# zengxianyu/sketchedit

Measured on AMD Instinct MI355X. Metric: images/sec, higher is better.
Workload: dtype f32; 1 GPU; SketchEdit inference forward (netM+netG, use_cam, pool max) 256x256 batch 32 per GPU, procedural weights; global_batch=32, size=256, per_gpu_batch=32, execution=default, two streams

## Files before the change

### sketchedit_amd/_lib.py

```python
import contextlib
import ctypes
import os
import subprocess
import threading

import numpy as np

_HERE = os.path.dirname(os.path.abspath(__file__))
LIB_PATH = os.environ.get("SKETCHEDIT_HIP_LIB") or os.path.join(_HERE, "lib", "libsketchedit_hip.so")
CSRC = os.path.join(_HERE, "csrc")
SOURCES = ["se_gconv.hip", "se_rconv16.hip", "se_rconv96.hip", "se_rtile.hip", "se_rtilew.hip", "se_wino.hip", "se_wino24.hip", "se_wino48.hip", "se_wino_up.hip", "se_wino_up48.hip", "se_attention.hip", "se_att_stream.hip", "se_misc.hip", "se_resize.hip",
           "se_window.hip", "se_feather.hip", "se_fill.hip", "se_select.hip", "se_lasso.hip", "se_modify.hip", "se_outline.hip", "se_move.hip", "se_warp.hip", "se_filter.hip", "se_adjust.hip", "se_png.hip", "se_jpg.hip", "se_pack.hip",
           "se_plan.hip", "se_api_window.hip", "se_api_select.hip", "se_api_move.hip", "se_api_codec.hip", "se_api_debug.hip", "se_api.hip"]

SE_NET_G, SE_NET_M = 0, 1
RESAMPLE_LANCZOS, RESAMPLE_BILINEAR, RESAMPLE_BICUBIC = 1, 2, 3
FLAG_USE_CAM, FLAG_POOL_MAX, FLAG_NO_MASK_CC, FLAG_NO_MASK_COARSE, FLAG_JOINT_TRAIN_INP = 1, 2, 4, 8, 16
FLAG_LOW_LATENCY, FLAG_GRAPH, FLAG_PACKED_OUT, FLAG_BF16, FLAG_CONSERVATIVE = 32, 64, 128, 256, 512
LOW_LATENCY_MAX_PIXELS = 3 * 256 * 256
LOW_LATENCY_MAX_SINGLE_IMAGE = 512 * 512

SYMBOLS = ["se_create", "se_destroy", "se_last_error", "se_version", "se_load_weights", "se_weights_ready",
           "se_workspace_bytes", "se_netM_forward", "se_netM_forward_ex", "se_netG_forward", "se_netG_forward_taps", "se_inference", "se_inference_u8", "se_gated_conv2d",
           "se_gated_conv2d_ex", "se_attention", "se_attention_ex", "se_quantize_u8", "se_dequantize_u8", "se_inference_u8io", "se_profile_enable",
# ... 301 lines not shown
        if device not in _shared:
            _shared[device] = Engine(device)
        return _shared[device]


def set_option(name, value):
    if load_library().se_debug_set_option(name.encode(), int(value)):
        raise SketchEditHipError("unknown developer switch %r" % name)


def get_option(name):
    v = ctypes.c_int(0)
    if load_library().se_debug_get_option(name.encode(), ctypes.byref(v)):
        raise SketchEditHipError("unknown developer switch %r" % name)
    return v.value


def reset_options():
    load_library().se_debug_reset_options()


def gconv_form(cin, cout, H, W, k=3, stride=1, rate=1, act="elu", upsample=False, cin1=0, x1_is_vector=False, B=1,
               low_latency=False, bf16=False, conservative=False, net=SE_NET_G):
    flags = (FLAG_LOW_LATENCY if low_latency else 0) | (FLAG_BF16 if bf16 else 0) | (FLAG_CONSERVATIVE if conservative else 0)
    buf = ctypes.create_string_buffer(64)
    fn = load_library().se_debug_gconv_form
    fn.argtypes, fn.restype = [ctypes.c_int] * 14 + [ctypes.c_char_p, ctypes.c_size_t], ctypes.c_int
    if fn(cin, cin1, int(bool(x1_is_vector)), cout, k, stride, rate, {"elu": 0, "relu": 1, None: 2}[act],
          int(bool(upsample)), B, H, W, flags, net, buf, len(buf)):
        raise SketchEditHipError("gconv_form: not a layer gated_conv2d takes")
    return buf.value.decode().split(",")


def flags_from_opt(opt):
    f = 0
    if getattr(opt, "use_cam", False):
        f |= FLAG_USE_CAM
    pool = getattr(opt, "pool_type", "avg")
    if pool == "max":
        f |= FLAG_POOL_MAX
    elif pool != "avg":
        raise NotImplementedError(pool)
    if getattr(opt, "no_mask_cc", False):
        f |= FLAG_NO_MASK_CC
    if getattr(opt, "no_mask_coarse", False):
        f |= FLAG_NO_MASK_COARSE
    if getattr(opt, "joint_train_inp", False):
        f |= FLAG_JOINT_TRAIN_INP
    return f


def _ptr(t):
    return None if t is None else ctypes.c_void_p(t.data_ptr())


def _check_dev(*ts):
    import torch
    for t in ts:
        if t is None:
            continue
        if not (isinstance(t, torch.Tensor) and t.is_cuda and t.dtype == torch.float32 and t.is_contiguous()):
            raise SketchEditHipError("expected contiguous float32 CUDA(HIP) tensors")


def upload_u8(a, device):
    import warnings
# ... 1070 lines not shown
```

### sketchedit_amd/csrc/se_api.hip

```cpp
#include "se_host.h"

using namespace se;

namespace se {

thread_local std::string g_create_err;

}

namespace {

void destroy_graph(se_ctx::GraphEntry& g) {
  if (g.exec) {
    if (g.stream) (void)hipStreamSynchronize(g.stream);
    (void)hipGraphExecDestroy(g.exec);
  }
  if (g.graph) (void)hipGraphDestroy(g.graph);
  g.exec = nullptr; g.graph = nullptr;
}
void drop_graphs(se_ctx* c) {
  for (auto& g : c->graphs) destroy_graph(g);
  c->graphs.clear();
}
void evict_lru_graph(se_ctx* c) {
// ... 46 lines not shown
  }
  t.last_use = ++c->rs_clock;
  c->rs_tables.push_back(std::move(t));
  return &c->rs_tables.back();
}

unsigned char* rs_scratch(se_ctx* c, size_t bytes) {
  if (bytes > c->rs_scratch_bytes) {
    if (c->rs_scratch) {
      (void)hipStreamSynchronize(c->rs_stream);
      (void)hipFree(c->rs_scratch);
      c->rs_scratch = nullptr; c->rs_scratch_bytes = 0;
    }
    const size_t sz = (bytes + ((size_t)1 << 20) - 1) & ~(((size_t)1 << 20) - 1);
    if (hipMalloc(&c->rs_scratch, sz) != hipSuccess) { c->rs_scratch = nullptr; fail(c, "resize: cannot allocate %zu bytes", sz); return nullptr; }
    c->rs_scratch_bytes = sz;
  }
  return c->rs_scratch;
}

int inference_u8_locked(se_ctx* c, void* stream, const float* image, const float* sketch, unsigned char* rgb_out,
                        unsigned char* mask_u8_out, void* ws, size_t ws_bytes, int B, int H, int W, int flags, int tail_planes,
                        const unsigned char* lock8) {
  flags &= ~(SE_FLAG_GRAPH | SE_FLAG_PACKED_OUT);
  const size_t plane = ((size_t)B * H * W * 4 + 255) & ~(size_t)255;
  const size_t tail = (2 + (size_t)tail_planes) * plane;
  if (ws_bytes < tail) return fail(c, "workspace too small: %zu bytes", ws_bytes);
  float* hard_all = (float*)((char*)ws + ws_bytes - tail + plane);
  float* soft_all = (float*)((char*)ws + ws_bytes - tail);
  const size_t HW = (size_t)H * W;
  const int nb = pass_size(c, B, H, W, flags);
  if (!nb) return 1;
  if (poison(c, soft_all, 2 * plane, (hipStream_t)stream)) return 1;
  for (int b0 = 0; b0 < B; b0 += nb) {
    const int bb = std::min(nb, B - b0);
    const se_ctx::Peaks pk = plan_peaks(c, 3, bb, H, W, flags, false);
    if (carve(c, pk, ws, ws_bytes, tail)) return 1;
    const float *img = image + b0 * 3 * HW, *sk = sketch + b0 * HW;
    float *hard = hard_all + b0 * HW, *soft = soft_all + b0 * HW;
    begin_call(c, stream, flags);
    int rc = plan_netM(c, img, sk, soft, hard, nullptr, bb, H, W, 0, lock8 ? lock8 + b0 * HW : nullptr);
    if (rc) return rc;
    if (carve(c, pk, ws, ws_bytes, tail)) return 1;
    c->rgb8 = rgb_out + b0 * 3 * HW; c->m8 = mask_u8_out ? mask_u8_out + b0 * HW : nullptr;
    rc = plan_netG(c, img, img, hard, hard, sk, nullptr, nullptr, soft, nullptr, bb, H, W, flags);
    if (rc) return rc;
  }
  return 0;
}

}

namespace {

int resize_locked(se_ctx* c, hipStream_t st, const unsigned char* in, int B, int Hin, int Win, int C, ResizeOut o, int Hout,
                  int Wout, int filter) {
  if (!in || (o.mode == RESIZE_OUT_U8 ? !o.u8 : !o.f32)) return fail(c, "null pointer argument");
  if (B < 1 || B > 65535 || Hin < 1 || Win < 1 || Hout < 1 || Wout < 1 || Hin > 65535 || Hout > 65535 || (C != 1 && C != 3))
    return fail(c, "resize: bad shape B=%d %dx%dx%d -> %dx%d (C in {1, 3}, heights and B < 65536)", B, Hin, Win, C, Hout, Wout);
  if (filter != SE_RESAMPLE_BILINEAR && filter != SE_RESAMPLE_BICUBIC && filter != SE_RESAMPLE_LANCZOS)
    return fail(c, "resize: unsupported filter %d", filter);
  if (o.mode == RESIZE_OUT_IMAGE_F32) o.lut = c->lut8;
  if (rs_enter(c, st)) return 1;
  set_profiler(&c->prof);
  o.H = Hout; o.W = Wout;
  const bool need_h = Win != Wout, need_v = Hin != Hout;
  if (!need_h && !need_v) {
    if (o.mode == RESIZE_OUT_U8) {
      HIPCHK(c, hipMemcpyAsync(o.u8, in, (size_t)B * Hin * Win * C, hipMemcpyDeviceToDevice, st));
      return 0;
    }
    if (((size_t)Hin * Win) % 4 || ((uintptr_t)in & 3) || ((uintptr_t)o.f32 & 15))
      return fail(c, "resize: an unresized fp32 output needs H W %% 4 == 0, a 4-byte aligned input and a 16-byte aligned output");
    if (o.mode == RESIZE_OUT_IMAGE_F32 && C == 3)
      HIPCHK(c, launch_dequantize_u8(in, nullptr, c->lut8, o.f32, nullptr, B, Hin, Win, st));
    else if (o.mode == RESIZE_OUT_SKETCH_F32 && C == 1)
      HIPCHK(c, launch_dequantize_u8(nullptr, in, c->lut8, nullptr, o.f32, B, Hin, Win, st));
    else
// ... 139 lines not shown
}

int se_weights_ready(se_ctx* c) {
  if (!c) return 0;
  std::lock_guard<std::mutex> lk(c->mu);
  for (auto* net : {&c->G, &c->M})
    for (auto& kv : *net)
      if (!kv.second.packed) return 0;
  return 1;
}

size_t se_workspace_bytes(se_ctx* c, int B, int H, int W) {
  if (!c) return 0;
  std::lock_guard<std::mutex> lk(c->mu);
  if (check_dims(c, B, H, W)) return 0;
  c->fork2 = opt(OPT_FORK_DEFAULT) != 0;
  size_t peak = 0;
  for (int cam = 0; cam < 2; ++cam)
    for (int joint = 0; joint < 2; ++joint)
      for (int ll = 0; ll < 2; ++ll)
        for (int bf = 0; bf < 2; ++bf) {
          const int flags = (cam ? SE_FLAG_USE_CAM : 0) | (joint ? SE_FLAG_JOINT_TRAIN_INP : 0) | (ll ? SE_FLAG_LOW_LATENCY : 0) |
                            (bf ? SE_FLAG_BF16 : 0) | SE_FLAG_POOL_MAX;
          const int nb = pass_size(c, B, H, W, flags);
          if (!nb) return 0;
          const int last = B % nb;
          for (int ser = 0; ser < 2; ++ser)
            for (int mi = 0; mi < 2; ++mi)
              for (int bb : {nb, last}) {
                if (!bb) continue;
                c->serial = ser != 0;
                const se_ctx::Peaks pk = plan_peaks(c, 3, bb, H, W, flags, mi != 0);
                if (pk.main + pk.side > peak) peak = pk.main + pk.side;
              }
          c->serial = false;
        }
  return peak + 6 * (((size_t)B * H * W * 4 + 255) & ~(size_t)255);
}

int se_netM_forward_ex(se_ctx* c, void* stream, const float* image, const float* sketch, float* mask_out,
                       float* maskim_out, void* ws, size_t ws_bytes, int B, int H, int W, int exec_flags) {
  if (!c) return 1;
  std::lock_guard<std::mutex> lk(c->mu);
  if (check_dims(c, B, H, W)) return 1;
  if (!image || !sketch || !mask_out || !ws) return fail(c, "null pointer argument");
  if (forward_enter(c)) return 1;
  exec_flags &= SE_FLAG_LOW_LATENCY | SE_FLAG_BF16 | SE_FLAG_CONSERVATIVE;
  const int nb = pass_size(c, B, H, W, exec_flags);
  if (!nb) return 1;
  const size_t HW = (size_t)H * W;
  for (int b0 = 0; b0 < B; b0 += nb) {
    const int bb = std::min(nb, B - b0);
    if (carve(c, plan_peaks(c, 1, bb, H, W, exec_flags, maskim_out != nullptr), ws, ws_bytes, 0)) return 1;
    begin_call(c, stream, exec_flags);
    const int rc = plan_netM(c, image + b0 * 3 * HW, sketch + b0 * HW, mask_out + b0 * HW, nullptr,
                             maskim_out ? maskim_out + b0 * 3 * HW : nullptr, bb, H, W);
    if (rc) return rc;
  }
  return 0;
}

int se_netM_forward(se_ctx* c, void* stream, const float* image, const float* sketch, float* mask_out,
                    float* maskim_out, void* ws, size_t ws_bytes, int B, int H, int W) {
  return se_netM_forward_ex(c, stream, image, sketch, mask_out, maskim_out, ws, ws_bytes, B, H, W, 0);
}

// ... 11 lines not shown
  const size_t HW = (size_t)H * W;
  for (int b0 = 0; b0 < B; b0 += nb) {
    const int bb = std::min(nb, B - b0);
    if (carve(c, plan_peaks(c, 2, bb, H, W, flags, false), ws, ws_bytes, 0)) return 1;
    begin_call(c, stream, flags);
    c->taps = taps;
    const int rc = plan_netG(c, x + b0 * 3 * HW, x2 + b0 * 3 * HW, mask + b0 * HW, mask2 + b0 * HW, guide + b0 * HW,
                             coarse_out ? coarse_out + b0 * 3 * HW : nullptr, fine_out + b0 * 3 * HW, nullptr, nullptr, bb, H, W, flags);
    c->taps = nullptr;
    if (rc) return rc;
  }
  return 0;
}

int se_netG_forward(se_ctx* c, void* stream, const float* x, const float* x2, const float* mask, const float* mask2,
                    const float* guide, float* coarse_out, float* fine_out, void* ws, size_t ws_bytes, int B, int H,
                    int W, int flags) {
  return se_netG_forward_taps(c, stream, x, x2, mask, mask2, guide, coarse_out, fine_out, ws, ws_bytes, B, H, W, flags, nullptr);
}

namespace {
int enqueue_inference(se_ctx* c, void* stream, const float* image, const float* sketch, float* composed_out, float* mask_out,
                      float* hard_out, float* maskim_out, float* coarse_out, float* fine_out, void* ws, size_t ws_bytes,
                      int B, int H, int W, int flags, const unsigned char* lock8 = nullptr) {
  const size_t plane = ((size_t)B * H * W * 4 + 255) & ~(size_t)255;
  float* hard_all = hard_out ? hard_out : (float*)((char*)ws + ws_bytes - plane);
  const size_t HW = (size_t)H * W;
  const long packed_bs = (flags & SE_FLAG_PACKED_OUT) ? 4l * H * W : 0;
  if (packed_bs) mask_out = composed_out + 3 * HW;
  const size_t comp_bs = packed_bs ? (size_t)packed_bs : 3 * HW, mask_bs = packed_bs ? (size_t)packed_bs : HW;
  const int nb = pass_size(c, B, H, W, flags);
  if (!nb) return 1;
  if (!hard_out && poison(c, hard_all, plane, (hipStream_t)stream)) return 1;
  for (int b0 = 0; b0 < B; b0 += nb) {
    const int bb = std::min(nb, B - b0);
    const se_ctx::Peaks pk = plan_peaks(c, 3, bb, H, W, flags, maskim_out != nullptr);
    if (carve(c, pk, ws, ws_bytes, plane)) return 1;
    const float *img = image + b0 * 3 * HW, *sk = sketch + b0 * HW;
    float *hard = hard_all + b0 * HW, *mk = mask_out + b0 * mask_bs;
    begin_call(c, stream, flags);
    int rc = plan_netM(c, img, sk, mk, hard, maskim_out ? maskim_out + b0 * 3 * HW : nullptr, bb, H, W, packed_bs,
                       lock8 ? lock8 + b0 * HW : nullptr);
    if (rc) return rc;
    if (carve(c, pk, ws, ws_bytes, plane)) return 1;
    rc = plan_netG(c, img, img, hard, hard, sk, coarse_out ? coarse_out + b0 * 3 * HW : nullptr, fine_out ? fine_out + b0 * 3 * HW : nullptr,
                   mk, composed_out + b0 * comp_bs, bb, H, W, flags, packed_bs);
    if (rc) return rc;
  }
  return 0;
}
}

int se_inference(se_ctx* c, void* stream, const float* image, const float* sketch, float* composed_out,
                 float* mask_out, float* hard_out, float* maskim_out, float* coarse_out, float* fine_out, void* ws,
                 size_t ws_bytes, int B, int H, int W, int flags) {
  if (!c) return 1;
  std::lock_guard<std::mutex> lk(c->mu);
  if (check_dims(c, B, H, W)) return 1;
  if (!image || !sketch || !composed_out || (!mask_out && !(flags & SE_FLAG_PACKED_OUT)) || !ws) return fail(c, "null pointer argument");
  if (forward_enter(c)) return 1;
  if (!(flags & SE_FLAG_GRAPH) || c->prof.on || poison_byte() != 0)
    return enqueue_inference(c, stream, image, sketch, composed_out, mask_out, hard_out, maskim_out, coarse_out, fine_out, ws,
                             ws_bytes, B, H, W, flags);
  const std::vector<long long> key = {(long long)(size_t)image, (long long)(size_t)sketch, (long long)(size_t)composed_out,
                                      (long long)(size_t)mask_out, (long long)(size_t)hard_out, (long long)(size_t)maskim_out,
                                      (long long)(size_t)coarse_out, (long long)(size_t)fine_out, (long long)(size_t)ws,
                                      (long long)ws_bytes, B, H, W, flags, opt_epoch()};
  se_ctx::GraphEntry* ge = nullptr;
  for (auto& g : c->graphs)
    if (g.key == key) { ge = &g; break; }
  if (!ge) {
    if (c->graphs.size() >= 16) evict_lru_graph(c);
    c->graphs.emplace_back();
    c->graphs.back().key = key;
    c->graphs.back().last_use = ++c->graph_clock;
    return enqueue_inference(c, stream, image, sketch, composed_out, mask_out, hard_out, maskim_out, coarse_out, fine_out, ws,
                             ws_bytes, B, H, W, flags);
  }
  ge->last_use = ++c->graph_clock;
// ... 165 lines not shown
```

### sketchedit_amd/csrc/se_api_debug.hip

```cpp
#include "se_host.h"

using namespace se;

extern "C" {

int se_profile_enable(se_ctx* c, int on) {
  if (!c) return 1;
  std::lock_guard<std::mutex> lk(c->mu);
  HIPCHK(c, hipSetDevice(c->device));
  c->prof.recs.clear();
  c->prof.used = 0;
  if (on && c->prof.pool.empty()) {
    c->prof.pool.resize(2 * 1024);
    for (auto& e : c->prof.pool) HIPCHK(c, hipEventCreate(&e));
  }
  c->prof.on = on != 0;
  return 0;
}

int se_profile_report(se_ctx* c, char* buf, size_t cap) {
  if (!c || !buf || cap < 64) return 1;
  std::lock_guard<std::mutex> lk(c->mu);
  HIPCHK(c, hipSetDevice(c->device));
  HIPCHK(c, hipDeviceSynchronize());
// ... 20 lines not shown
  std::map<std::string, long> cnt;
  for (auto& r : c->prof.recs) {
    if (!r.name) continue;
    float t = 0.f;
    if (hipEventElapsedTime(&t, r.a, r.b) != hipSuccess) continue;
    std::string k = std::string(prof_label_name(r.label)) + ":" + r.name;
    if (!cnt.count(k)) keys.push_back(k);
    agg[k].first += t; agg[k].second += r.flops; aggx[k] += r.exec_flops; cnt[k]++;
  }
  first = true;
  for (auto& k : keys) {
    char t[384];
    snprintf(t, sizeof t, "%s{\"layer\": \"%s\", \"launches\": %ld, \"total_ms\": %.6f, \"flops\": %.6e, \"flops_executed\": %.6e}",
             first ? "" : ", ", k.c_str(), cnt[k], agg[k].first, agg[k].second, aggx[k]);
    s += t;
    first = false;
  }
  s += "], \"launches\": [";
  first = true;
  for (auto& r : c->prof.recs) {
    char t[256];
    snprintf(t, sizeof t, "%s{\"form\": \"%s\", \"kernel\": \"%s\", \"layer\": \"%s\", \"workgroups\": %ld}", first ? "" : ", ",
             r.form ? r.form : "?", prof_label_name(r.label), r.name ? r.name : "", r.blocks);
    s += t;
    first = false;
  }
  s += "]}";
  if (s.size() + 1 > cap) return fail(c, "profile buffer too small");
  memcpy(buf, s.c_str(), s.size() + 1);
  return 0;
}

int se_debug_set_option(const char* name, int value) { return opt_set(name, value); }
int se_debug_get_option(const char* name, int* value) { return opt_get(name, value); }
void se_debug_reset_options(void) { opt_reset(); }

int se_debug_gconv_form(int cin, int cin1, int src1_is_vector, int cout, int k, int stride, int rate, int act, int upsample,
                        int B, int H, int W, int exec_flags, int net_id, char* out, size_t cap) {
  if (!out || cin <= 0 || cin1 < 0 || cout <= 0 || k <= 0 || stride <= 0 || rate <= 0 || B <= 0 || H <= 0 || W <= 0) return 1;
  const bool bf = (exec_flags & SE_FLAG_BF16) != 0;
  const int gran = bf ? 8 : 4;
  if (cin1 && ((cin % gran) || (cin1 % gran))) return 1;
  const LayerDef d = {"test", cin + cin1, cout, k, stride, rate, act, upsample};
  const bool raw = small_layer(d);
  if (raw && (k != 3 || cin != 12 || cin1 || (cout != 1 && cout != 3) || stride != 1 || rate != 1 || upsample)) return 1;
  if (!raw && (cout % 8)) return 1;
  const LayerFacts f = layer_facts(d, cin + cin1);
  if (!raw && f.cfg < 0) return 1;
  const int Cp = (cin + gran - 1) & ~(gran - 1);
  if (!raw && Cp + cin1 != f.CG[bf] * gran) return 1;
  const bool vec = cin1 && src1_is_vector;
  const ConvCall q = {d, f, B, H, W, Cp, cin1, cin1 ? (vec ? SRC2_VECTOR : SRC2_TENSOR) : SRC2_NONE, bf,
                      (exec_flags & SE_FLAG_LOW_LATENCY) != 0, (exec_flags & SE_FLAG_CONSERVATIVE) != 0, net_id, vec};
  const Choice ch = choose_form(q);
  const char* name = form_name(ch, q);
  if (!name) return 1;
  const std::string s = std::string(ch.fold ? "vecbias," : "") + name;
  if (s.size() + 1 > cap) return 1;
  memcpy(out, s.c_str(), s.size() + 1);
  return 0;
}

int se_gated_conv2d_ex(se_ctx* c, void* stream, const float* x, const float* x1, int x1_is_vector, const float* w_host,
                       const float* b_host, float* y, int B, int Cin, int Cin1, int H, int W, int Cout, int k, int stride,
                       int rate, int act, int upsample, int exec_flags) {
  if (!c || !x || !w_host || !b_host || !y) return 1;
  std::lock_guard<std::mutex> lk(c->mu);
// ... 202 lines not shown
```

### sketchedit_amd/csrc/se_host.h

```cpp
#pragma once
#include "../../include/sketchedit_hip.h"
#include "se_kernels.h"
#include "se_pack.h"

#include <cstdarg>
#include <cstdint>
#include <cstdlib>
#include <cstdio>
#include <cstring>
#include <algorithm>
#include <map>
#include <mutex>
#include <numeric>
#include <string>
#include <vector>

namespace se {

struct Arena {
  struct Blk { size_t off, size; bool used; };
  std::vector<Blk> blks;
  size_t cap = 0, peak = 0;
  bool dry = false;
  char* base = nullptr;
// ... 26 lines not shown
    for (size_t i = 0; i < blks.size(); ++i) {
      if (blks[i].off == off && blks[i].used) {
        blks[i].used = false;
        if (i + 1 < blks.size() && !blks[i + 1].used) { blks[i].size += blks[i + 1].size; blks.erase(blks.begin() + i + 1); }
        if (i > 0 && !blks[i - 1].used) { blks[i - 1].size += blks[i].size; blks.erase(blks.begin() + i); }
        return;
      }
    }
  }
};

}

struct se_ctx {
  int device = 0;
  std::mutex mu;
  std::string err;
  std::map<std::string, se::Layer> G, M;
  se::Layer wconv1_j4;
  float* zeros = nullptr;
  float* lut8 = nullptr;
  se::Arena arena;
  se::Arena arena2;
  hipStream_t st = nullptr;
  hipStream_t st_main = nullptr;
  hipStream_t st_side = nullptr;
  hipEvent_t ev_fork = nullptr, ev_join = nullptr;
  bool dry = false;
  bool low_latency = false;
  int cur_net = SE_NET_G;
  bool bf16 = false;
  bool serial = false;
  bool fork2 = true;
  bool conservative = false;
  const se_netG_taps* taps = nullptr;
  float* vbias_ws = nullptr;
  const float* vec32 = nullptr;
  unsigned char* rgb8 = nullptr;
  unsigned char* m8 = nullptr;
  se::Profiler prof;
  struct Peaks { size_t main, side; };
  std::map<std::vector<long long>, Peaks> peaks;
  size_t dry_max_act = 0;
  std::map<std::vector<long long>, long long> act_per_img;
  struct GraphEntry {
    std::vector<long long> key;
    hipGraph_t graph = nullptr;
    hipGraphExec_t exec = nullptr;
    hipStream_t stream = nullptr;
    unsigned long long last_use = 0;
  };
  unsigned long long graph_clock = 0;
  std::vector<GraphEntry> graphs;
  struct ResampleTable {
    int in, out, filter, ksize;
    std::vector<int> host;
    int* dev = nullptr;
    unsigned long long last_use = 0;
  };
  std::vector<ResampleTable> rs_tables;
  unsigned long long rs_clock = 0;
  unsigned char* rs_scratch = nullptr;
  size_t rs_scratch_bytes = 0;
  hipStream_t rs_stream = nullptr;
  bool rs_used = false;
  hipEvent_t rs_event = nullptr;
// ... 36 lines not shown
inline int poison_byte() {
  const int v = opt(OPT_TEST_POISON);
  return v >= 1 && v <= 255 ? v : 0;
}
inline int poison(se_ctx* c, void* p, size_t bytes, hipStream_t st) {
  const int v = poison_byte();
  if (!v || !p || !bytes) return 0;
  HIPCHK(c, hipMemsetAsync(p, v, bytes, st));
  return 0;
}

inline bool aligned_to(const void* p, int a) { return ((uintptr_t)p & (uintptr_t)(a - 1)) == 0; }

inline size_t pad256(size_t n) { return (n + 255) & ~(size_t)255; }

inline bool overlaps(const void* a, size_t an, const void* b, size_t bn) {
  return (uintptr_t)a < (uintptr_t)b + bn && (uintptr_t)b < (uintptr_t)a + an;
}

inline int check_dims(se_ctx* c, int B, int H, int W) {
  if (B < 1 || H < 16 || W < 16 || (H % 8) || (W % 8)) return fail(c, "bad shape B=%d H=%d W=%d (H, W must be multiples of 8, >= 16)", B, H, W);
  return 0;
}

inline void begin_call(se_ctx* c, void* stream, int flags) {
  c->st = c->st_main = (hipStream_t)stream;
  c->dry = false;
  c->low_latency = (flags & SE_FLAG_LOW_LATENCY) != 0;
  c->bf16 = (flags & SE_FLAG_BF16) != 0;
  c->conservative = (flags & SE_FLAG_CONSERVATIVE) != 0;
  c->serial = c->prof.on;
  c->taps = nullptr;
  c->rgb8 = nullptr; c->m8 = nullptr;
  c->cur_net = SE_NET_G;
  set_profiler(&c->prof);
}

inline int forward_enter(se_ctx* c) {
  HIPCHK(c, hipSetDevice(c->device));
  c->serial = c->prof.on;
  c->fork2 = opt(OPT_FORK_DEFAULT) != 0;
  return 0;
}

inline int device_enter(se_ctx* c) {
  HIPCHK(c, hipSetDevice(c->device));
  set_profiler(&c->prof);
  return 0;
}

extern const LayerDef G_LAYERS[], M_LAYERS[];
extern const int NG, NM;

int run_gconv(se_ctx* c, const Layer& L, const float* src0, int C0, const float* src1, int C1, int src1_vec, float* dst,
              int B, int Hin, int Win);

struct Act {
  float* p = nullptr;
  int H = 0, W = 0, C = 0;
};

struct Plan {
  se_ctx* c;
  std::map<std::string, Layer>& net;
  int B;
  int rc = 0;
  Arena* ar;
  Plan(se_ctx* c_, std::map<std::string, Layer>& n, int B_) : c(c_), net(n), B(B_), ar(&c_->arena) {}
  float* alloc_raw(size_t nfloats) {
    float* p = ar->alloc(nfloats);
    if (!p && !rc) rc = fail(c, "workspace too small (need more than %zu bytes)", ar->cap);
    if (p && !rc && !c->dry && poison(c, p, (nfloats * 4 + 255) & ~(size_t)255, c->st)) rc = 1;
    return p;
  }
  Act alloc(int H, int W, int C) {
    Act a; a.H = H; a.W = W;
    if (c->bf16) {
      a.C = (C + 7) & ~7;
      a.p = alloc_raw(((size_t)B * H * W * a.C + 1) / 2);
    } else {
      a.C = C;
      a.p = alloc_raw((size_t)B * H * W * C);
    }
    if (c->dry) c->dry_max_act = std::max(c->dry_max_act, (size_t)B * H * W * a.C * (c->bf16 ? 2 : 4));
    return a;
  }
  void release(const float* p) {
    if (!p) return;
    if (c->arena2.owns(p)) c->arena2.release(p); else c->arena.release(p);
  }
  void free(Act& a) { release(a.p); a.p = nullptr; }
  bool forked() const { return (c->low_latency || (c->fork2 && !c->serial)) && c->st_side; }
  int side_begin() {
    if (!forked()) return 0;
    ar = &c->arena2;
    if (c->dry) return 0;
    HIPCHK(c, hipEventRecord(c->ev_fork, c->st_main));
    HIPCHK(c, hipStreamWaitEvent(c->st_side, c->ev_fork, 0));
    c->st = c->st_side;
    return 0;
  }
  int side_end() {
    if (!forked()) return 0;
    ar = &c->arena;
    if (c->dry) return 0;
    HIPCHK(c, hipEventRecord(c->ev_join, c->st_side));
    c->st = c->st_main;
    return 0;
  }
  int join() {
    if (!forked() || c->dry) return 0;
    HIPCHK(c, hipStreamWaitEvent(c->st_main, c->ev_join, 0));
    return 0;
  }
  Act conv(const char* name, Act& in, bool rel = true, const float* src1 = nullptr, int C1 = 0, int vec = 0) {
    if (rc) return Act();
    return conv_layer(net.at(name), in, rel, src1, C1, vec);
  }
  Act conv_layer(Layer& L, Act& in, bool rel = true, const float* src1 = nullptr, int C1 = 0, int vec = 0) {
    Act out;
    if (rc) return out;
    const ConvShape sh = conv_shape(L.def, in.H, in.W);
    out = alloc(sh.Ho, sh.Wo, L.def.cout / 2);
    if (rc) return out;
    if (!c->dry) rc = run_gconv(c, L, in.p, in.C, src1, C1, vec, out.p, B, in.H, in.W);
    if (rel) free(in);
    return out;
  }
};

int plan_netM(se_ctx* c, const float* image, const float* sketch, float* mask_out, float* hard_out, float* maskim_out,
              int B, int H, int W, long packed_bs = 0, const unsigned char* lock = nullptr);
int plan_netG(se_ctx* c, const float* x, const float* x2, const float* mask, const float* mask2, const float* guide,
              float* coarse_out, float* fine_out, const float* soft_mask, float* composed_out, int B, int H, int W,
              int flags, long packed_bs = 0);
int att_row_stride(int R, bool bf);
bool att_streaming(int h, int w, bool bf, bool want_similar);
int run_attention(se_ctx* c, Plan& P, Act& x, const float* mask_full, Act& out, float* similar_nchw);
int pass_size(se_ctx* c, int B, int H, int W, int flags);
se_ctx::Peaks plan_peaks(se_ctx* c, int which, int B, int H, int W, int flags, bool want_maskim);
int carve(se_ctx* c, const se_ctx::Peaks& pk, void* ws, size_t ws_bytes, size_t tail);

int rs_enter(se_ctx* c, hipStream_t st);
const se_ctx::ResampleTable* rs_table(se_ctx* c, int in, int out, int filter);
unsigned char* rs_scratch(se_ctx* c, size_t bytes);
int inference_u8_locked(se_ctx* c, void* stream, const float* image, const float* sketch, unsigned char* rgb_out,
                        unsigned char* mask_u8_out, void* ws, size_t ws_bytes, int B, int H, int W, int flags, int tail_planes,
                        const unsigned char* lock8 = nullptr);

int win_check_records(se_ctx* c, const se_window* wins, int B, int hs, int ws, bool need_sketch);
const se_window* win_put(se_ctx* c, hipStream_t st, const se_window* wins, int B);

}
```

### sketchedit_amd/csrc/se_kernels.h

```cpp
#pragma once
#include <hip/hip_runtime.h>
#include <stddef.h>
#include <stdint.h>

#include <vector>

struct se_window;

namespace se {

enum ProfLabel { PL_GCONV_N192 = 0, PL_GCONV_N96, PL_GCONV_N48, PL_GCONV_N24, PL_WINO_N192, PL_WINO_N96, PL_WINO_UP96, PL_SMALL_CONV, PL_PACK, PL_COLREDUCE,
                 PL_ATT_PREP, PL_ATT_SCORE, PL_ATT_SOFTMAX, PL_ATT_BOXSUM, PL_ATT_PV, PL_LAYOUT,
                 PL_ATT_STREAM_STATS, PL_ATT_STREAM_OUT, PL_RESIZE_H, PL_RESIZE_V, PL_WINDOW_GATHER, PL_WINDOW_BORDER, PL_WINDOW_PASTE,
                 PL_WINDOW_RESAMPLE_H, PL_WINDOW_PASTE_V, PL_WINDOW_SAVE, PL_WINDOW_SWAP, PL_WINDOW_LOCK_GATHER, PL_WINDOW_PASTE_LOCKED,
                 PL_WINDOW_PASTE_V_LOCKED, PL_SKETCH_TILES, PL_SKETCH_STROKES, PL_PNG_ROWS, PL_PNG_STRIPES,
                 PL_PNG_FINISH, PL_JPG_BLOCKS, PL_JPG_ROWS, PL_JPG_FINISH, PL_JPG2_BLOCKS, PL_JPG2_HIST, PL_JPG2_TABLES,
                 PL_WINDOW_PASTE_FEATHER, PL_FILL_MASKS, PL_FILL_KEEP, PL_SELECT_SIMILAR, PL_SELECT_FLOOD, PL_SELECT_GROW, PL_MODIFY_DISC, PL_MODIFY_VOTE,
                 PL_LASSO_FILL, PL_PLANE_COMBINE, PL_ADJUST, PL_HIST_TILES, PL_HIST_SUM, PL_ADJUST_LUT, PL_OUTLINE_COUNT, PL_OUTLINE_SCAN, PL_OUTLINE_EMIT, PL_FILTER_BLUR, PL_FILTER_MOSAIC, PL_MOVE_DROP,
                 PL_PLANE_SHIFT, PL_WARP_DROP, PL_PLANE_WARP, PL_COUNT };
const char* prof_label_name(int l);
struct Profiler {
  struct Rec { int label; const char* name; const char* form; double flops; double exec_flops; double bytes; long blocks; hipEvent_t a, b; };
  std::vector<Rec> recs;
  std::vector<hipEvent_t> pool;
  size_t used = 0;
  bool on = false;
};
void set_profiler(Profiler* p);
void set_launch_cost(double flops, double bytes, const char* name = nullptr, double exec_flops = -1.0);
void set_launch_grid(long blocks);
hipError_t ensure_max_lds(const void* func, int bytes);

#define SE_OPTIONS(X)                                                                                         \
  X(XCD_REMAP, 1)                                                             \
  X(RTILE, 1)                                              \
  X(RTILE_LL_MIN, 256)         \
  X(RTILE_WX, 2)          \
  X(RTILE_DENSE, 1)                                          \
  X(RTILE_D5W, 1)                                        \
  X(TEST_OFFSET_LIMIT, 0)  \
  X(TEST_POISON, 0)       \
  X(RCONV16, 1) X(RCONV16_DUAL, 1) X(RCONV96, 1) X(VECBIAS, 1)                                                  \
  X(WINOGRAD, 1) X(WINOGRAD48, 1) X(WINOGRAD_UP, 1) X(WINOGRAD_UP48, 1)                                         \
  X(WINOGRAD_F43, 1)      \
  X(GCONV_FAST, 1) X(FORK_DEFAULT, 1) X(LL_WINO_MIN_WG, 64) X(LL_WINO48_MIN_WG, 128)                            \
  X(ATT_FUSED, -1) X(ATT_FUSED_BF16, -1) X(ATT_PTILDE_LDS, 1) X(ATT_STATS_LDS, 1) X(ATT_E16, 1) X(ATT_SYM, 1)   \
  X(ATT_STREAM, 0)
enum Opt {
#define X(name, dflt) OPT_##name,
  SE_OPTIONS(X)
#undef X
  OPT_COUNT
};
int opt(int o);
int opt_set(const char* name, int value);
int opt_get(const char* name, int* value);
void opt_reset();
long long opt_epoch();

struct GConvParams {
  const float* src0;
  const float* src1;
  const float* wpk;
  const float* bias;
  float* dst;
  const float* zeros;
  int B, Hin, Win, Ho, Wo;
  int C0, C1;
  int C0g, CG;
  int T, KW;
  int magicCG, magicKW;
  int magicKH;
  unsigned rep;
  unsigned div_hw_m, div_w_m;
  int div_hw_l, div_w_l;
  int stride, dil, pad;
  int ushift;
  int up2;
  int OH, OW;
  int Hlim, Wlim;
// ... 282 lines not shown
```

### sketchedit_amd/csrc/se_plan.hip

```cpp
#include "se_host.h"

#include <numeric>

using namespace se;

namespace {

#define ENC(p)                                                                                    \
  {p "2_downsample", 24, 96, 3, 2, 1, ACT_ELU, 0}, {p "3", 48, 96, 3, 1, 1, ACT_ELU, 0},          \
      {p "4_downsample", 48, 192, 3, 2, 1, ACT_ELU, 0}, {p "5", 96, 192, 3, 1, 1, ACT_ELU, 0},    \
      {p "6", 96, 192, 3, 1, 1, ACT_ELU, 0}, {p "7_atrous", 96, 192, 3, 1, 2, ACT_ELU, 0},        \
      {p "8_atrous", 96, 192, 3, 1, 4, ACT_ELU, 0}, {p "9_atrous", 96, 192, 3, 1, 8, ACT_ELU, 0}, \
      {p "10_atrous", 96, 192, 3, 1, 16, ACT_ELU, 0}
#define DEC(p, c11in, c17out)                                                                        \
  {p "11", c11in, 192, 3, 1, 1, ACT_ELU, 0}, {p "12", 96, 192, 3, 1, 1, ACT_ELU, 0},                 \
      {p "13_upsample_conv", 96, 96, 3, 1, 1, ACT_ELU, 1}, {p "14", 48, 96, 3, 1, 1, ACT_ELU, 0},    \
      {p "15_upsample_conv", 48, 48, 3, 1, 1, ACT_ELU, 1}, {p "16", 24, 24, 3, 1, 1, ACT_ELU, 0},    \
      {p "17", 12, c17out, 3, 1, 1, ACT_NONE, 0}

}

namespace se {

const LayerDef G_LAYERS[] = {
// ... 298 lines not shown
  return 0;
}

}

namespace se {

int plan_netM(se_ctx* c, const float* image, const float* sketch, float* mask_out, float* hard_out, float* maskim_out,
              int B, int H, int W, long packed_bs, const unsigned char* lock) {
  Plan P(c, c->M, B);
  c->cur_net = SE_NET_M;
  Act in = P.alloc(H, W, 4);
  if (P.rc) return P.rc;
  if (!c->dry) HIPCHK(c, c->bf16 ? launch_pack_m16(image, sketch, in.p, B, H, W, c->st) : launch_pack_m(image, sketch, in.p, B, H, W, c->st));
  Act x9;
  const bool want_img = maskim_out != nullptr;
  Act x10 = encoder(P, "conv", in, want_img ? &x9 : nullptr);
  if (want_img) {
    Act d = decoder(P, "conv", x9);
    small(P, "conv17", d, 1, maskim_out, nullptr, nullptr, nullptr, nullptr, nullptr, 0);
  }
  Act d = decoder(P, "conv_mask_", x10);
  small(P, "conv_mask_17", d, 0, mask_out, hard_out, nullptr, nullptr, nullptr, nullptr, 0, packed_bs, lock);
  return P.rc;
}

int plan_netG(se_ctx* c, const float* x, const float* x2, const float* mask, const float* mask2, const float* guide,
              float* coarse_out, float* fine_out, const float* soft_mask, float* composed_out, int B, int H, int W,
              int flags, long packed_bs) {
  Plan P(c, c->G, B);
  c->cur_net = SE_NET_G;
  const int joint = (flags & SE_FLAG_JOINT_TRAIN_INP) ? 1 : 0;
  Act cin = P.alloc(H, W, 8);
  P.ar = P.forked() ? &c->arena2 : &c->arena;
  Act sin = P.alloc(H, W, joint ? 4 : 8);
  P.ar = &c->arena;
  if (P.rc) return P.rc;
  if (!c->dry)
    HIPCHK(c, (c->bf16 ? launch_pack_g16 : launch_pack_g)(x, x2, mask, mask2, guide, cin.p, sin.p, B, H, W,
                                                          (flags & SE_FLAG_NO_MASK_CC) ? 1 : 0, joint, c->st));
  if (P.side_begin()) return 1;
  Act xs = encoder(P, "wconv", sin, nullptr, joint ? &c->wconv1_j4 : nullptr);
  Act part = P.alloc(1, COLREDUCE_SPLITS, 192), vec32 = P.alloc(1, 1, 192), vec = P.alloc(1, 1, 96);
  if (P.rc) return P.rc;
  if (!c->dry)
    HIPCHK(c, launch_colreduce(xs.p, part.p, c->bf16 ? vec32.p : vec.p, B, xs.H * xs.W, 96, (flags & SE_FLAG_POOL_MAX) ? 0 : 1,
                               c->st, c->bf16 ? 1 : 0, c->bf16 ? vec.p : nullptr));
  if (!c->dry && c->taps && c->taps->style_vec)
    HIPCHK(c, hipMemcpyAsync(c->taps->style_vec, c->bf16 ? vec32.p : vec.p, (size_t)B * 96 * 4, hipMemcpyDeviceToDevice, c->st));
  P.free(xs);
  P.free(part);
  if (!c->bf16) P.free(vec32);
  if (P.side_end()) return 1;
  Act xc = encoder(P, "conv", cin, nullptr);
  if (P.rc) return P.rc;
  if (P.join()) return 1;
  float* vb = P.alloc_raw((size_t)B * 9 * 192);
  if (P.rc) return P.rc;
  c->vbias_ws = vb;
  c->vec32 = c->bf16 ? vec32.p : nullptr;
  Act d = decoder(P, "conv", xc, vec.p, 96, 1);
  c->vbias_ws = nullptr; c->vec32 = nullptr;
  P.release(vb);
  if (c->bf16) P.free(vec32);
  P.free(vec);
  Act xnow = P.alloc(H, W, 4);
  if (P.rc) return P.rc;
  small(P, "conv17", d, 2, coarse_out, nullptr, x, mask, xnow.p, nullptr, (flags & SE_FLAG_NO_MASK_COARSE) ? 1 : 0);
  if (P.rc) return P.rc;
// ... 86 lines not shown
    AttParams a;
    memset(&a, 0, sizeof a);
    a.x = x.p; a.rn = rn; a.xn = xn; a.hard = mask_full; a.out = out.p;
    a.B = B; a.h = h; a.w = w; a.hs = hs; a.ws = ws; a.L = L; a.Lp = Lp;
    a.scale = 10.f; a.th = 0.1f;
    if (stream) {
      a.hc = hc; a.wc = wc; a.R = R; a.Rp = Rp; a.bf16 = bf ? 1 : 0;
      a.validR = valid; a.kmul = valid + (size_t)B * Rp; a.kadd = valid + 2 * (size_t)B * Rp;
      a.xT = xT; a.stats = stats;
      HIPCHK(c, launch_attention_stream(a, c->st));
    } else {
      a.hc = hc; a.wc = wc; a.R = R; a.Rp = Rp; a.bf16 = bf ? 1 : 0;
      a.validR = valid + guard; a.xT = xT; a.E = S + guard; a.P = S2; a.stats = stats; a.guard = guard; a.similar = similar_nchw;
      a.kmul = valid + ((size_t)B * Rp + guard) + guard; a.kadd = valid + 2 * ((size_t)B * Rp + guard) + guard;
      a.kadd2 = valid + 3 * ((size_t)B * Rp + guard) + guard; a.ea4 = valid + 4 * ((size_t)B * Rp + guard) + guard;
      a.ea = valid + 5 * ((size_t)B * Rp + guard) + guard; a.eb = valid + 6 * ((size_t)B * Rp + guard) + guard;
      a.emean = valid + 7 * ((size_t)B * Rp + guard); a.epart = a.emean + (size_t)B * 768;
      HIPCHK(c, launch_attention(a, c->st));
    }
  }
  P.release(S2); P.release(S); P.release(xT); P.release(stats); P.release(valid);
  P.release(xn); P.release(rn); P.release(part);
  return 0;
}

}

namespace {

long long max_act_bytes_per_image(se_ctx* c, int H, int W, int flags) {
  const std::vector<long long> key = {H, W, (flags & SE_FLAG_BF16) ? 1 : 0};
  auto it = c->act_per_img.find(key);
  if (it != c->act_per_img.end()) return it->second;
  const bool dry0 = c->dry, ll0 = c->low_latency, bf0 = c->bf16;
  c->dry = true; c->low_latency = false; c->bf16 = (flags & SE_FLAG_BF16) != 0;
  c->dry_max_act = 0;
  float dummy;
  c->arena.reset(nullptr, 0, true, 0); c->arena2.reset(nullptr, 0, true, 1);
  plan_netM(c, nullptr, nullptr, nullptr, nullptr, &dummy, 1, H, W, 0);
  c->arena.reset(nullptr, 0, true, 0); c->arena2.reset(nullptr, 0, true, 1);
  plan_netG(c, nullptr, nullptr, nullptr, nullptr, nullptr, nullptr, nullptr, nullptr, nullptr, 1, H, W, SE_FLAG_USE_CAM | SE_FLAG_POOL_MAX, 0);
  c->dry = dry0; c->low_latency = ll0; c->bf16 = bf0;
  const long long v = (long long)c->dry_max_act;
  c->act_per_img[key] = v;
  return v;
}

}

namespace se {

int pass_size(se_ctx* c, int B, int H, int W, int flags) {
  const long long per_img = max_act_bytes_per_image(c, H, W, flags);
  const long long lim = addr_limit();
  if (per_img <= 0) { fail(c, "internal: no activation size for %dx%d", H, W); return 0; }
  if (per_img >= lim) {
    fail(c, "a %dx%d image exceeds the kernels' 32-bit byte offsets (%lld bytes per activation, limit %lld)", H, W, per_img, lim);
    return 0;
  }
  const long long bmax = (lim - 1) / per_img;
  if (B <= bmax) return B;
  const long long passes = (B + bmax - 1) / bmax;
  return (int)((B + passes - 1) / passes);
}

se_ctx::Peaks plan_peaks(se_ctx* c, int which, int B, int H, int W, int flags, bool want_maskim) {
  const std::vector<long long> key = {which, B, H, W,
                                      flags & (SE_FLAG_USE_CAM | SE_FLAG_JOINT_TRAIN_INP | SE_FLAG_LOW_LATENCY | SE_FLAG_BF16),
                                      want_maskim ? 1 : 0, c->fork2 ? 1 : 0, opt_epoch(), c->serial ? 1 : 0};
  auto it = c->peaks.find(key);
  if (it != c->peaks.end()) return it->second;
  const bool dry0 = c->dry, ll0 = c->low_latency, bf0 = c->bf16;
  c->dry = true;
  c->low_latency = (flags & SE_FLAG_LOW_LATENCY) != 0;
  c->bf16 = (flags & SE_FLAG_BF16) != 0;
  float dummy;
  se_ctx::Peaks pk{0, 0};
  if (which & 1) {
    c->arena.reset(nullptr, 0, true, 0); c->arena2.reset(nullptr, 0, true, 1);
    plan_netM(c, nullptr, nullptr, nullptr, nullptr, want_maskim ? &dummy : nullptr, B, H, W);
    pk.main = c->arena.peak; pk.side = c->arena2.peak;
  }
  if (which & 2) {
    c->arena.reset(nullptr, 0, true, 0); c->arena2.reset(nullptr, 0, true, 1);
    plan_netG(c, nullptr, nullptr, nullptr, nullptr, nullptr, nullptr, nullptr, nullptr, nullptr, B, H, W, flags);
    if (c->arena.peak > pk.main) pk.main = c->arena.peak;
    if (c->arena2.peak > pk.side) pk.side = c->arena2.peak;
  }
  c->dry = dry0; c->low_latency = ll0; c->bf16 = bf0;
  c->peaks[key] = pk;
  return pk;
}

int carve(se_ctx* c, const se_ctx::Peaks& pk, void* ws, size_t ws_bytes, size_t tail) {
  if (ws_bytes < pk.main + pk.side + tail)
    return fail(c, "workspace too small: %zu bytes, this call needs %zu", ws_bytes, pk.main + pk.side + tail);
  c->arena.reset((char*)ws, ws_bytes - tail - pk.side, false);
  c->arena2.reset((char*)ws + (ws_bytes - tail - pk.side), pk.side, false);
  return 0;
}

}
```

Measured before the change: 2968 images/sec.

## Split large batches into two halves run concurrently on main and side streams

When a pass has enough pixels (batch*H*W at or above a threshold, default 2M) and low-latency mode is off, the batch is split into two halves. One half runs netM+netG on the main stream with the main arena, the other on the side stream with the side arena, joined by events. The per-layer intra-network fork is disabled in this paired mode. The goal is better GPU occupancy from two independent streams of work, at the cost of smaller per-kernel batches and a larger workspace split across the two arenas.

```diff
diff --git a/sketchedit_amd/_lib.py b/sketchedit_amd/_lib.py
--- a/sketchedit_amd/_lib.py
+++ b/sketchedit_amd/_lib.py
@@ -357,6 +357,14 @@
     return buf.value.decode().split(",")
 
 
+def pair_rule(B, H, W, low_latency=False):
+    v = ctypes.c_int(-1)
+    name = "SE_PAIR_RULE:%d,%d,%d,%d" % (B, H, W, FLAG_LOW_LATENCY if low_latency else 0)
+    if load_library().se_debug_get_option(name.encode(), ctypes.byref(v)):
+        raise SketchEditHipError("pair_rule: bad shape B=%d H=%d W=%d" % (B, H, W))
+    return bool(v.value)
+
+
 def flags_from_opt(opt):
     f = 0
     if getattr(opt, "use_cam", False):
diff --git a/sketchedit_amd/csrc/se_api.hip b/sketchedit_amd/csrc/se_api.hip
--- a/sketchedit_amd/csrc/se_api.hip
+++ b/sketchedit_amd/csrc/se_api.hip
@@ -102,18 +102,26 @@
   const int nb = pass_size(c, B, H, W, flags);
   if (!nb) return 1;
   if (poison(c, soft_all, 2 * plane, (hipStream_t)stream)) return 1;
-  for (int b0 = 0; b0 < B; b0 += nb) {
-    const int bb = std::min(nb, B - b0);
-    const se_ctx::Peaks pk = plan_peaks(c, 3, bb, H, W, flags, false);
+  for (int p0 = 0; p0 < B; p0 += nb) {
+    const int pb = std::min(nb, B - p0);
+    const bool pair = pair_pass(c, pb, H, W, flags);
+    const se_ctx::Peaks pk = plan_peaks(c, 3, pb, H, W, flags, false, pair);
     if (carve(c, pk, ws, ws_bytes, tail)) return 1;
-    const float *img = image + b0 * 3 * HW, *sk = sketch + b0 * HW;
-    float *hard = hard_all + b0 * HW, *soft = soft_all + b0 * HW;
-    begin_call(c, stream, flags);
-    int rc = plan_netM(c, img, sk, soft, hard, nullptr, bb, H, W, 0, lock8 ? lock8 + b0 * HW : nullptr);
-    if (rc) return rc;
-    if (carve(c, pk, ws, ws_bytes, tail)) return 1;
-    c->rgb8 = rgb_out + b0 * 3 * HW; c->m8 = mask_u8_out ? mask_u8_out + b0 * HW : nullptr;
-    rc = plan_netG(c, img, img, hard, hard, sk, nullptr, nullptr, soft, nullptr, bb, H, W, flags);
+    if (pair && pair_fork(c, (hipStream_t)stream)) return 1;
+    int rc = 0;
+    for (int half = 0; half < (pair ? 2 : 1) && !rc; ++half) {
+      const int b0 = p0 + (half ? pair_first(pb) : 0), bb = !pair ? pb : half ? pb - pair_first(pb) : pair_first(pb);
+      const float *img = image + b0 * 3 * HW, *sk = sketch + b0 * HW;
+      float *hard = hard_all + b0 * HW, *soft = soft_all + b0 * HW;
+      begin_call(c, stream, flags);
+      if (pair) pair_half(c, half);
+      rc = plan_netM(c, img, sk, soft, hard, nullptr, bb, H, W, 0, lock8 ? lock8 + b0 * HW : nullptr);
+      if (!rc) rc = carve(c, pk, ws, ws_bytes, tail);
+      if (rc) break;
+      c->rgb8 = rgb_out + b0 * 3 * HW; c->m8 = mask_u8_out ? mask_u8_out + b0 * HW : nullptr;
+      rc = plan_netG(c, img, img, hard, hard, sk, nullptr, nullptr, soft, nullptr, bb, H, W, flags);
+    }
+    if (pair && pair_join(c, (hipStream_t)stream) && !rc) rc = 1;
     if (rc) return rc;
   }
   return 0;
@@ -319,6 +327,10 @@
                 c->serial = ser != 0;
                 const se_ctx::Peaks pk = plan_peaks(c, 3, bb, H, W, flags, mi != 0);
                 if (pk.main + pk.side > peak) peak = pk.main + pk.side;
+                if (pair_pass(c, bb, H, W, flags)) {
+                  const se_ctx::Peaks pp = plan_peaks(c, 3, bb, H, W, flags, mi != 0, true);
+                  if (pp.main + pp.side > peak) peak = pp.main + pp.side;
+                }
               }
           c->serial = false;
         }
@@ -396,19 +408,27 @@
   const int nb = pass_size(c, B, H, W, flags);
   if (!nb) return 1;
   if (!hard_out && poison(c, hard_all, plane, (hipStream_t)stream)) return 1;
-  for (int b0 = 0; b0 < B; b0 += nb) {
-    const int bb = std::min(nb, B - b0);
-    const se_ctx::Peaks pk = plan_peaks(c, 3, bb, H, W, flags, maskim_out != nullptr);
+  for (int p0 = 0; p0 < B; p0 += nb) {
+    const int pb = std::min(nb, B - p0);
+    const bool pair = pair_pass(c, pb, H, W, flags);
+    const se_ctx::Peaks pk = plan_peaks(c, 3, pb, H, W, flags, maskim_out != nullptr, pair);
     if (carve(c, pk, ws, ws_bytes, plane)) return 1;
-    const float *img = image + b0 * 3 * HW, *sk = sketch + b0 * HW;
-    float *hard = hard_all + b0 * HW, *mk = mask_out + b0 * mask_bs;
-    begin_call(c, stream, flags);
-    int rc = plan_netM(c, img, sk, mk, hard, maskim_out ? maskim_out + b0 * 3 * HW : nullptr, bb, H, W, packed_bs,
-                       lock8 ? lock8 + b0 * HW : nullptr);
-    if (rc) return rc;
-    if (carve(c, pk, ws, ws_bytes, plane)) return 1;
-    rc = plan_netG(c, img, img, hard, hard, sk, coarse_out ? coarse_out + b0 * 3 * HW : nullptr, fine_out ? fine_out + b0 * 3 * HW : nullptr,
-                   mk, composed_out + b0 * comp_bs, bb, H, W, flags, packed_bs);
+    if (pair && pair_fork(c, (hipStream_t)stream)) return 1;
+    int rc = 0;
+    for (int half = 0; half < (pair ? 2 : 1) && !rc; ++half) {
+      const int b0 = p0 + (half ? pair_first(pb) : 0), bb = !pair ? pb : half ? pb - pair_first(pb) : pair_first(pb);
+      const float *img = image + b0 * 3 * HW, *sk = sketch + b0 * HW;
+      float *hard = hard_all + b0 * HW, *mk = mask_out + b0 * mask_bs;
+      begin_call(c, stream, flags);
+      if (pair) pair_half(c, half);
+      rc = plan_netM(c, img, sk, mk, hard, maskim_out ? maskim_out + b0 * 3 * HW : nullptr, bb, H, W, packed_bs,
+                     lock8 ? lock8 + b0 * HW : nullptr);
+      if (!rc) rc = carve(c, pk, ws, ws_bytes, plane);
+      if (rc) break;
+      rc = plan_netG(c, img, img, hard, hard, sk, coarse_out ? coarse_out + b0 * 3 * HW : nullptr, fine_out ? fine_out + b0 * 3 * HW : nullptr,
+                     mk, composed_out + b0 * comp_bs, bb, H, W, flags, packed_bs);
+    }
+    if (pair && pair_join(c, (hipStream_t)stream) && !rc) rc = 1;
     if (rc) return rc;
   }
   return 0;
diff --git a/sketchedit_amd/csrc/se_api_debug.hip b/sketchedit_amd/csrc/se_api_debug.hip
--- a/sketchedit_amd/csrc/se_api_debug.hip
+++ b/sketchedit_amd/csrc/se_api_debug.hip
@@ -76,7 +76,16 @@
 }
 
 int se_debug_set_option(const char* name, int value) { return opt_set(name, value); }
-int se_debug_get_option(const char* name, int* value) { return opt_get(name, value); }
+int se_debug_get_option(const char* name, int* value) {
+  static const char q[] = "SE_PAIR_RULE:";
+  if (name && value && !strncmp(name, q, sizeof q - 1)) {
+    int B = 0, H = 0, W = 0, flags = 0, end = 0;
+    if (sscanf(name + sizeof q - 1, "%d,%d,%d,%d%n", &B, &H, &W, &flags, &end) != 4 || name[sizeof q - 1 + end] || B < 1 || H < 1 || W < 1) return 1;
+    *value = pair_rule(B, H, W, flags) ? 1 : 0;
+    return 0;
+  }
+  return opt_get(name, value);
+}
 void se_debug_reset_options(void) { opt_reset(); }
 
 int se_debug_gconv_form(int cin, int cin1, int src1_is_vector, int cout, int k, int stride, int rate, int act, int upsample,
diff --git a/sketchedit_amd/csrc/se_host.h b/sketchedit_amd/csrc/se_host.h
--- a/sketchedit_amd/csrc/se_host.h
+++ b/sketchedit_amd/csrc/se_host.h
@@ -82,6 +82,8 @@
   bool bf16 = false;
   bool serial = false;
   bool fork2 = true;
+  bool paired = false;
+  int half = 0;
   bool conservative = false;
   const se_netG_taps* taps = nullptr;
   float* vbias_ws = nullptr;
@@ -184,6 +186,7 @@
   c->serial = c->prof.on;
   c->taps = nullptr;
   c->rgb8 = nullptr; c->m8 = nullptr;
+  c->paired = false; c->half = 0;
   c->cur_net = SE_NET_G;
   set_profiler(&c->prof);
 }
@@ -218,7 +221,8 @@
   int B;
   int rc = 0;
   Arena* ar;
-  Plan(se_ctx* c_, std::map<std::string, Layer>& n, int B_) : c(c_), net(n), B(B_), ar(&c_->arena) {}
+  Plan(se_ctx* c_, std::map<std::string, Layer>& n, int B_) : c(c_), net(n), B(B_), ar(home()) {}
+  Arena* home() const { return c->paired && c->half ? &c->arena2 : &c->arena; }
   float* alloc_raw(size_t nfloats) {
     float* p = ar->alloc(nfloats);
     if (!p && !rc) rc = fail(c, "workspace too small (need more than %zu bytes)", ar->cap);
@@ -242,7 +246,7 @@
     if (c->arena2.owns(p)) c->arena2.release(p); else c->arena.release(p);
   }
   void free(Act& a) { release(a.p); a.p = nullptr; }
-  bool forked() const { return (c->low_latency || (c->fork2 && !c->serial)) && c->st_side; }
+  bool forked() const { return !c->paired && (c->low_latency || (c->fork2 && !c->serial)) && c->st_side; }
   int side_begin() {
     if (!forked()) return 0;
     ar = &c->arena2;
@@ -290,7 +294,18 @@
 bool att_streaming(int h, int w, bool bf, bool want_similar);
 int run_attention(se_ctx* c, Plan& P, Act& x, const float* mask_full, Act& out, float* similar_nchw);
 int pass_size(se_ctx* c, int B, int H, int W, int flags);
-se_ctx::Peaks plan_peaks(se_ctx* c, int which, int B, int H, int W, int flags, bool want_maskim);
+inline bool pair_rule(int bb, int H, int W, int flags) {
+  const int min_pixels = opt(OPT_PAIR_MIN_PIXELS);
+  return !(flags & SE_FLAG_LOW_LATENCY) && bb >= 2 && min_pixels > 0 && (long long)bb * H * W >= min_pixels;
+}
+inline int pair_first(int bb) { return (bb + 1) / 2; }
+inline bool pair_pass(const se_ctx* c, int bb, int H, int W, int flags) {
+  return pair_rule(bb, H, W, flags) && !c->serial && !c->taps && c->st_side;
+}
+se_ctx::Peaks plan_peaks(se_ctx* c, int which, int B, int H, int W, int flags, bool want_maskim, bool pair = false);
+int pair_fork(se_ctx* c, hipStream_t main);
+void pair_half(se_ctx* c, int half);
+int pair_join(se_ctx* c, hipStream_t main);
 int carve(se_ctx* c, const se_ctx::Peaks& pk, void* ws, size_t ws_bytes, size_t tail);
 
 int rs_enter(se_ctx* c, hipStream_t st);
diff --git a/sketchedit_amd/csrc/se_kernels.h b/sketchedit_amd/csrc/se_kernels.h
--- a/sketchedit_amd/csrc/se_kernels.h
+++ b/sketchedit_amd/csrc/se_kernels.h
@@ -45,7 +45,8 @@
   X(WINOGRAD_F43, 1)      \
   X(GCONV_FAST, 1) X(FORK_DEFAULT, 1) X(LL_WINO_MIN_WG, 64) X(LL_WINO48_MIN_WG, 128)                            \
   X(ATT_FUSED, -1) X(ATT_FUSED_BF16, -1) X(ATT_PTILDE_LDS, 1) X(ATT_STATS_LDS, 1) X(ATT_E16, 1) X(ATT_SYM, 1)   \
-  X(ATT_STREAM, 0)
+  X(ATT_STREAM, 0)        \
+  X(PAIR_MIN_PIXELS, 1 << 21)
 enum Opt {
 #define X(name, dflt) OPT_##name,
   SE_OPTIONS(X)
diff --git a/sketchedit_amd/csrc/se_plan.hip b/sketchedit_amd/csrc/se_plan.hip
--- a/sketchedit_amd/csrc/se_plan.hip
+++ b/sketchedit_amd/csrc/se_plan.hip
@@ -354,9 +354,9 @@
   c->cur_net = SE_NET_G;
   const int joint = (flags & SE_FLAG_JOINT_TRAIN_INP) ? 1 : 0;
   Act cin = P.alloc(H, W, 8);
-  P.ar = P.forked() ? &c->arena2 : &c->arena;
+  P.ar = P.forked() ? &c->arena2 : P.home();
   Act sin = P.alloc(H, W, joint ? 4 : 8);
-  P.ar = &c->arena;
+  P.ar = P.home();
   if (P.rc) return P.rc;
   if (!c->dry)
     HIPCHK(c, (c->bf16 ? launch_pack_g16 : launch_pack_g)(x, x2, mask, mask2, guide, cin.p, sin.p, B, H, W,
@@ -509,15 +509,15 @@
   const std::vector<long long> key = {H, W, (flags & SE_FLAG_BF16) ? 1 : 0};
   auto it = c->act_per_img.find(key);
   if (it != c->act_per_img.end()) return it->second;
-  const bool dry0 = c->dry, ll0 = c->low_latency, bf0 = c->bf16;
-  c->dry = true; c->low_latency = false; c->bf16 = (flags & SE_FLAG_BF16) != 0;
+  const bool dry0 = c->dry, ll0 = c->low_latency, bf0 = c->bf16, pair0 = c->paired;
+  c->dry = true; c->low_latency = false; c->bf16 = (flags & SE_FLAG_BF16) != 0; c->paired = false;
   c->dry_max_act = 0;
   float dummy;
   c->arena.reset(nullptr, 0, true, 0); c->arena2.reset(nullptr, 0, true, 1);
   plan_netM(c, nullptr, nullptr, nullptr, nullptr, &dummy, 1, H, W, 0);
   c->arena.reset(nullptr, 0, true, 0); c->arena2.reset(nullptr, 0, true, 1);
   plan_netG(c, nullptr, nullptr, nullptr, nullptr, nullptr, nullptr, nullptr, nullptr, nullptr, 1, H, W, SE_FLAG_USE_CAM | SE_FLAG_POOL_MAX, 0);
-  c->dry = dry0; c->low_latency = ll0; c->bf16 = bf0;
+  c->dry = dry0; c->low_latency = ll0; c->bf16 = bf0; c->paired = pair0;
   const long long v = (long long)c->dry_max_act;
   c->act_per_img[key] = v;
   return v;
@@ -541,32 +541,54 @@
   return (int)((B + passes - 1) / passes);
 }
 
-se_ctx::Peaks plan_peaks(se_ctx* c, int which, int B, int H, int W, int flags, bool want_maskim) {
+se_ctx::Peaks plan_peaks(se_ctx* c, int which, int B, int H, int W, int flags, bool want_maskim, bool pair) {
   const std::vector<long long> key = {which, B, H, W,
                                       flags & (SE_FLAG_USE_CAM | SE_FLAG_JOINT_TRAIN_INP | SE_FLAG_LOW_LATENCY | SE_FLAG_BF16),
-                                      want_maskim ? 1 : 0, c->fork2 ? 1 : 0, opt_epoch(), c->serial ? 1 : 0};
+                                      want_maskim ? 1 : 0, c->fork2 ? 1 : 0, opt_epoch(), c->serial ? 1 : 0, pair ? 1 : 0};
   auto it = c->peaks.find(key);
   if (it != c->peaks.end()) return it->second;
-  const bool dry0 = c->dry, ll0 = c->low_latency, bf0 = c->bf16;
+  const bool dry0 = c->dry, ll0 = c->low_latency, bf0 = c->bf16, pair0 = c->paired;
+  const int half0 = c->half;
   c->dry = true;
   c->low_latency = (flags & SE_FLAG_LOW_LATENCY) != 0;
   c->bf16 = (flags & SE_FLAG_BF16) != 0;
   float dummy;
   se_ctx::Peaks pk{0, 0};
-  if (which & 1) {
-    c->arena.reset(nullptr, 0, true, 0); c->arena2.reset(nullptr, 0, true, 1);
-    plan_netM(c, nullptr, nullptr, nullptr, nullptr, want_maskim ? &dummy : nullptr, B, H, W);
-    pk.main = c->arena.peak; pk.side = c->arena2.peak;
-  }
-  if (which & 2) {
-    c->arena.reset(nullptr, 0, true, 0); c->arena2.reset(nullptr, 0, true, 1);
-    plan_netG(c, nullptr, nullptr, nullptr, nullptr, nullptr, nullptr, nullptr, nullptr, nullptr, B, H, W, flags);
-    if (c->arena.peak > pk.main) pk.main = c->arena.peak;
-    if (c->arena2.peak > pk.side) pk.side = c->arena2.peak;
-  }
-  c->dry = dry0; c->low_latency = ll0; c->bf16 = bf0;
+  for (int half = 0; half < (pair ? 2 : 1); ++half) {
+    const int nb = !pair ? B : half ? B - pair_first(B) : pair_first(B);
+    c->paired = pair; c->half = half;
+    if (which & 1) {
+      c->arena.reset(nullptr, 0, true, 0); c->arena2.reset(nullptr, 0, true, 1);
+      plan_netM(c, nullptr, nullptr, nullptr, nullptr, want_maskim ? &dummy : nullptr, nb, H, W);
+      if (c->arena.peak > pk.main) pk.main = c->arena.peak;
+      if (c->arena2.peak > pk.side) pk.side = c->arena2.peak;
+    }
+    if (which & 2) {
+      c->arena.reset(nullptr, 0, true, 0); c->arena2.reset(nullptr, 0, true, 1);
+      plan_netG(c, nullptr, nullptr, nullptr, nullptr, nullptr, nullptr, nullptr, nullptr, nullptr, nb, H, W, flags);
+      if (c->arena.peak > pk.main) pk.main = c->arena.peak;
+      if (c->arena2.peak > pk.side) pk.side = c->arena2.peak;
+    }
+  }
+  c->dry = dry0; c->low_latency = ll0; c->bf16 = bf0; c->paired = pair0; c->half = half0;
   c->peaks[key] = pk;
   return pk;
+}
+
+int pair_fork(se_ctx* c, hipStream_t main) {
+  HIPCHK(c, hipEventRecord(c->ev_fork, main));
+  HIPCHK(c, hipStreamWaitEvent(c->st_side, c->ev_fork, 0));
+  return 0;
+}
+void pair_half(se_ctx* c, int half) {
+  c->paired = true; c->half = half;
+  c->st = half ? c->st_side : c->st_main;
+}
+int pair_join(se_ctx* c, hipStream_t main) {
+  c->paired = false; c->half = 0; c->st = main;
+  HIPCHK(c, hipEventRecord(c->ev_join, c->st_side));
+  HIPCHK(c, hipStreamWaitEvent(main, c->ev_join, 0));
+  return 0;
 }
 
 int carve(se_ctx* c, const se_ctx::Peaks& pk, void* ws, size_t ws_bytes, size_t tail) {
```

Result: faster. 3011 images/sec (median of 6 runs) (+1.5%).
